# cosmodesi/desilike

Measured on AMD Instinct MI355X. Metric: log-likelihood evals/sec (full-shape P_ell, 3x40 bins), higher is better.
Workload: dtype f64; 1 GPU; BASELINE configs[1]: ShapeFit+Kaiser P_ell ell=(0,2,4) x 40 k-bins, dense window 120x1200 (n_kin=400/ell), 120x120 precision, 1024 batched param points per GPU per step; batch_per_gpu=1024, n_params=6, parallelism=walkers x1, collective=none, ranks=1

## Files before the change

### desilike_amd/csrc/dl_api.hip

```cpp
#include <hip/hip_runtime.h>
#include <chrono>
#include <thread>

#include <algorithm>
#include <cmath>
#include <cstdio>
#include <cstdlib>
#include <string>
#include <vector>

#include "../../include/desilike_amd.h"
#include "dl_host.hpp"
#include "dl_kernels.h"
#include "dl_ens_fold.h"
#include "dl_prior.h"
#include "dl_sample_solved.h"
#include "dl_sample_solved_data.h"
#include "dl_data_batch.h"
#include "dl_data_batch_marg.h"

static thread_local std::string g_last_error;
void dl_set_last_error(const char* msg) { g_last_error = msg ? msg : ""; }

struct DlWhitenHost {
// ... 132 lines not shown
    if (ctx) ctx->last_error = msg;
    g_last_error = msg;
    return 1;
}

template <typename T>
static int dl_upload(dl_ctx* ctx, T** dst, const std::vector<T>& src) {
    size_t bytes = std::max<size_t>(src.size(), 1) * sizeof(T);
    DL_HIP_CHECK(ctx, hipMalloc((void**)dst, bytes));
    if (!src.empty()) DL_HIP_CHECK(ctx, hipMemcpy(*dst, src.data(), src.size() * sizeof(T), hipMemcpyHostToDevice));
    return 0;
}

static_assert(sizeof(DlObsDev) <= 4096, "DlObsDev travels in the kernarg segment (4 KiB)");

extern "C" {

dl_config* dl_config_new(void) { return new dl_config(); }

int dl_config_set_f64(dl_config* cfg, const char* key, const double* data, int64_t n) {
    if (!cfg || !key || (n > 0 && !data) || n < 0) { g_last_error = "dl_config_set_f64: invalid argument"; return 1; }
    cfg->f64[key] = std::vector<double>(data, data + n);
    return 0;
}

int dl_config_set_i32(dl_config* cfg, const char* key, const int32_t* data, int64_t n) {
    if (!cfg || !key || (n > 0 && !data) || n < 0) { g_last_error = "dl_config_set_i32: invalid argument"; return 1; }
    cfg->i32[key] = std::vector<int32_t>(data, data + n);
    return 0;
}
// ... 270 lines not shown
                for (int k = 0; k < K; ++k) sum += wrow[k] * dvec[k];
                tconst[(size_t)s_ * ctx->N_pad + i] = sum;
            }
        }
        if (dl_upload(ctx, &ctx->tconst_dev, tconst)) { dl_destroy(ctx); return 1; }
        ctx->marg.tconst = ctx->tconst_dev;
    }
    if (dl_upload(ctx, &ctx->arena_dev, arena.data)) { dl_destroy(ctx); return 1; }
    for (auto& gf : gfrag_host) {
        double* dev = nullptr;
        if (dl_upload(ctx, &dev, gf)) { dl_destroy(ctx); return 1; }
        ctx->gfrag_dev.push_back(dev);
    }
    ctx->obs_kernarg.resize(ctx->n_obs);
    for (int i = 0; i < ctx->n_obs; ++i) { ctx->obs[i].rebase(ctx->arena_dev); ctx->obs_kernarg[i] = ctx->obs[i].dev; }
    if (dl_upload(ctx, &ctx->obs_array_dev, ctx->obs_kernarg)) { dl_destroy(ctx); return 1; }
    {
        size_t nbytes = (16384 / 32 + 8 + 64) * sizeof(int32_t);
        if (hipMalloc((void**)&ctx->gemm_counters, nbytes) != hipSuccess || hipMemset(ctx->gemm_counters, 0, nbytes) != hipSuccess) { dl_fail(ctx, "dl_create: counter allocation failed"); dl_destroy(ctx); return 1; }
        ctx->step_ready = ctx->gemm_counters + (16384 / 32 + 8);
    }
    {
        std::vector<double> frag((size_t)ctx->N_pad * ctx->K_pad);
        const int nks = ctx->K_pad / 4;
        for (int nt = 0; nt < ctx->N_pad / 16; ++nt)
            for (int ks = 0; ks < nks; ++ks)
                for (int lane = 0; lane < 64; ++lane)
                    frag[((size_t)nt * nks + ks) * 64 + lane] = wt_white[(size_t)(16 * nt + (lane & 15)) * ctx->K_pad + 4 * ks + (lane >> 4)];
        if (dl_upload(ctx, &ctx->wt_frag_dev, frag)) { dl_destroy(ctx); return 1; }
    }
    if (dl_upload(ctx, &ctx->priors_dev, priors) || dl_upload(ctx, &ctx->wt_white_dev, wt_white) ||
// ... 83 lines not shown
    const size_t R = 1 + ctx->n_var;
    DL_HIP_CHECK(ctx, hipMalloc((void**)&ctx->power_ws, (size_t)need * R * ctx->K_pad * sizeof(double)));
    DL_HIP_CHECK(ctx, hipMalloc((void**)&ctx->delta_ws, std::max<size_t>(2 * (size_t)need * R, (size_t)need * R + 16384 + 2048) * ctx->N_pad * sizeof(double)));
    DL_HIP_CHECK(ctx, hipMalloc((void**)&ctx->flat_ws, (size_t)need * ctx->N_pad * sizeof(double)));
    if (ctx->feat_ok) DL_HIP_CHECK(ctx, hipMalloc((void**)&ctx->feat_ws, (size_t)need * ctx->feat_ld * sizeof(double)));
    DL_HIP_CHECK(ctx, hipMalloc((void**)&ctx->stencil_ws, (size_t)need * ctx->n_params * sizeof(double)));
    DL_HIP_CHECK(ctx, hipMalloc((void**)&ctx->prior_rec_ws, (size_t)need * 2 * sizeof(double)));
    if (ctx->ws_ld > 0) {
        DL_HIP_CHECK(ctx, hipMalloc((void**)&ctx->ws_scratch, (size_t)need * ctx->ws_ld * sizeof(double)));
        DL_HIP_CHECK(ctx, hipMemset(ctx->ws_scratch, 0, (size_t)need * ctx->ws_ld * sizeof(double)));
        for (int i = 0; i < ctx->n_obs; ++i) {
            if (ctx->obs[i].dev.templ != 5) continue;
            ctx->obs_kernarg[i].coef_w = ctx->ws_scratch + ctx->obs[i].ws_col;
            ctx->obs_kernarg[i].n_band = (int32_t)ctx->ws_ld;
        }
        DL_HIP_CHECK(ctx, hipMemcpy(ctx->obs_array_dev, ctx->obs_kernarg.data(), ctx->obs_kernarg.size() * sizeof(DlObsDev), hipMemcpyHostToDevice));
    }
    DL_HIP_CHECK(ctx, hipMemset(ctx->power_ws, 0, (size_t)need * R * ctx->K_pad * sizeof(double)));
    DL_HIP_CHECK(ctx, hipMemset(ctx->delta_ws, 0, std::max<size_t>(2 * (size_t)need * R, (size_t)need * R + 16384 + 2048) * ctx->N_pad * sizeof(double)));
    DL_HIP_CHECK(ctx, hipMemset(ctx->flat_ws, 0, (size_t)need * ctx->N_pad * sizeof(double)));
    if (ctx->feat_ok) DL_HIP_CHECK(ctx, hipMemset(ctx->feat_ws, 0, (size_t)need * ctx->feat_ld * sizeof(double)));
    DL_HIP_CHECK(ctx, hipMemset(ctx->stencil_ws, 0, (size_t)need * ctx->n_params * sizeof(double)));
    DL_HIP_CHECK(ctx, hipMemset(ctx->prior_rec_ws, 0, (size_t)need * 2 * sizeof(double)));
    DL_HIP_CHECK(ctx, hipDeviceSynchronize());
    ctx->cap = need;
    return 0;
}

struct DlDataEval {
    const int32_t* index;
    double* out;
// ... 253 lines not shown
    DL_HIP_CHECK(ctx, hipSetDevice(ctx->device));
    if (dl_order_streams(ctx, stream)) return 1;
    const int64_t per_pass = std::max<int64_t>(1, DL_CHUNK / S);
    if (dl_reserve(ctx, std::min<int64_t>(B, per_pass) * S)) return 1;
    for (int64_t b0 = 0; b0 < B; b0 += per_pass) {
        const int64_t nc = std::min<int64_t>(per_pass, B - b0), nb = nc * S;
        const double* steps = steps_dev + (size_t)b0 * P * 2;
        dl_launch_fisher_stencil(centers_dev + (size_t)b0 * P, steps, P, nc, ctx->stencil_ws, stream);
        const double* th = ctx->stencil_ws;
        int n_slabs = 1, cps = 0;
        int64_t slab_stride = 0;
        const double* bias = nullptr;
        const bool emu_fused_env = !dl_options().no_emu_fused;
        const bool emu_fused = emu_fused_env || ctx->any_stacked;
        if (ctx->feat_ok) {
            if (!emu_fused) dl_launch_fullshape(ctx->obs_kernarg.data(), ctx->n_obs, th, P, nb, ctx->power_ws, ctx->K_pad, nullptr, 0, stream, ctx->feat_ws, ctx->feat_ld, 0);
            for (int i = 0; i < ctx->n_obs; ++i) {
                if (ctx->stk_steps[i]) dl_launch_emulated_stacked(ctx->obs_kernarg[i], th, P, nb, ctx->gfrag_dev[i], ctx->delta_ws, ctx->N_pad, ctx->N_pad, i > 0, ctx->stk_steps[i], stream, nullptr, nullptr, nullptr, 0, dl_stk_basis_ws(ctx, i));
                else if (emu_fused) dl_launch_emulated_feature(ctx->obs_kernarg[i], th, P, nb, ctx->gfrag_dev[i], ctx->delta_ws, ctx->N_pad, ctx->N_pad, i > 0, stream);
                else dl_launch_feature_gemm(ctx->feat_ws, ctx->feat_ld, ctx->obs_kernarg[i].feat_off, ctx->obs_kernarg[i].nb_pad, 1, ctx->gfrag_dev[i], ctx->delta_ws, ctx->N_pad,
                                            ctx->N_pad, nb, i > 0, stream);
            }
            bias = ctx->bias_white_dev;
        } else {
            dl_launch_fullshape(ctx->obs_kernarg.data(), ctx->n_obs, th, P, nb, ctx->power_ws, ctx->K_pad, nullptr, 0, stream, nullptr, 0, 0, ctx->obs_array_dev);
            if (ctx->any_transform) {
                dl_launch_window_gemm(ctx->power_ws, ctx->K_pad, ctx->wt_full_dev, ctx->K_pad, ctx->bias_full_dev, ctx->flat_ws, ctx->N_pad, nb, ctx->N_pad, ctx->N_pad, ctx->K_pad, 1, stream);
                dl_launch_transform(ctx->flat_ws, ctx->N_pad, ctx->flatdata_dev, ctx->transform_dev, n, nb, stream);
                dl_launch_window_gemm(ctx->flat_ws, ctx->N_pad, ctx->wh_dev, ctx->N_pad, ctx->bias_wh_dev, ctx->delta_ws, ctx->N_pad, nb, ctx->N_pad, ctx->N_pad, ctx->N_pad, 1, stream);
            } else {
                n_slabs = dl_gemm_tiled_splits(nb, ctx->N_pad, ctx->K_pad, &cps);
// ... 244 lines not shown
        ctx->grad_cap = 0;
        const int64_t cap = std::max<int64_t>((need + 63) / 64 * 64, 256);
        DL_HIP_CHECK(ctx, hipMalloc((void**)&ctx->eg_u, (size_t)cap * K * sizeof(double)));
        DL_HIP_CHECK(ctx, hipMalloc((void**)&ctx->eg_v, (size_t)cap * K * sizeof(double)));
        DL_HIP_CHECK(ctx, hipMalloc((void**)&ctx->eg_q, (size_t)cap * (1 + ctx->n_var) * DL_N_MONO * sizeof(double)));
        DL_HIP_CHECK(ctx, hipMalloc((void**)&ctx->eg_gb, std::max<size_t>(2 * (size_t)cap, (size_t)cap + 16384 + 2048) * ctx->eg_ngt * sizeof(double)));
        DL_HIP_CHECK(ctx, hipMalloc((void**)&ctx->grad_status, (size_t)cap * sizeof(int32_t)));
        DL_HIP_CHECK(ctx, hipMemset(ctx->eg_v, 0, (size_t)cap * K * sizeof(double)));
        DL_HIP_CHECK(ctx, hipDeviceSynchronize());
        ctx->eg_cap = cap;
    }
    for (int64_t b0 = 0; b0 < B; b0 += per_pass) {
        const int64_t nb = std::min<int64_t>(per_pass, B - b0);
        const double* th = theta_dev + (size_t)b0 * P;
        int32_t* st = status_dev ? status_dev + b0 : ctx->grad_status;
        dl_launch_fullshape(ctx->obs_kernarg.data(), 1, th, P, nb, ctx->power_ws, ctx->K_pad, nullptr, 0, stream, ctx->feat_ws, ctx->feat_ld, 0, nullptr);
        dl_launch_emu_grad_u(ctx->feat_ws, ctx->feat_ld, o.feat_off, o.nb_pad, ctx->gfrag_dev[0], ctx->eg_u, Np, Np, nb, stream);
        dl_launch_emu_grad_adjoint(ctx->feat_ws, ctx->feat_ld, o.feat_off, o.nb_pad, ctx->n_var, ctx->eg_u, Np, Np, ctx->bias_white_dev, ctx->marg, th, P, ctx->priors_dev,
                                   logposterior_dev + b0, st, ctx->eg_v, ctx->eg_q, nb, stream);
        int cps = 0;
        const int n_slabs = dl_gemm_tiled_splits(nb, ctx->eg_ngt, (int)K, &cps);
        const int64_t slab_stride = nb * (int64_t)ctx->eg_ngt;
        dl_launch_window_gemm_tiled(ctx->eg_v, K, ctx->eg_gt, K, ctx->eg_gb, slab_stride, ctx->eg_ngt, nb, ctx->eg_ngt, (int)K, n_slabs, cps, stream, 0);
        dl_launch_emu_grad_backprop(o, th, P, ctx->priors_dev, ctx->eg_gb, ctx->eg_ngt, n_slabs, slab_stride, ctx->eg_q, st, ctx->eg_wt, grad_dev + (size_t)b0 * P, nb, stream);
    }
    DL_HIP_CHECK(ctx, hipGetLastError());
    return 0;
}

int dl_eval_logposterior_grad(dl_ctx* ctx, const double* theta_dev, int64_t B, double* logposterior_dev, double* grad_dev, int32_t* status_dev, void* hip_stream) {
    if (!ctx) { g_last_error = "dl_eval_logposterior_grad: null context"; return 1; }
// ... 52 lines not shown
        dl_launch_fullshape_grad(ctx->obs_kernarg.data(), ctx->n_obs, ctx->obs_array_dev, th, P, nb, ctx->grad_y, Kp, ctx->grad_phys, ctx->priors_dev, st, grad_dev + (size_t)b0 * P, stream);
    }
    DL_HIP_CHECK(ctx, hipGetLastError());
    return 0;
}

int dl_eval_theory(dl_ctx* ctx, const double* theta_dev, int64_t B, int32_t iobs, double* power_dev, double* tables_dev, void* hip_stream) {
    if (!ctx) { g_last_error = "dl_eval_theory: null context"; return 1; }
    if (iobs < 0 || iobs >= ctx->n_obs) return dl_fail(ctx, "dl_eval_theory: observable index out of range");
    if (B < 0 || (B > 0 && (!theta_dev || !power_dev))) return dl_fail(ctx, "dl_eval_theory: invalid argument");
    if (B == 0) return 0;
    hipStream_t stream = (hipStream_t)hip_stream;
    DL_HIP_CHECK(ctx, hipSetDevice(ctx->device));
    const bool ws = ctx->obs_kernarg[iobs].templ == 5;
    if (ws && dl_reserve(ctx, B)) return 1;
    DlObsDev tmp = ctx->obs_kernarg[iobs];
    tmp.col_offset = 0;
    tmp.n_pass = 0;
    tmp.n_var = 0;
    for (int c = 0; c < DL_N_VPARS; ++c) tmp.vp_slot[c] = -1;
    for (int c = 0; c < DL_MAX_EFT; ++c) tmp.marg_ct_slot[c][0] = tmp.marg_ct_slot[c][1] = -1;
    if (dl_order_streams(ctx, stream)) return 1;
    for (int64_t b0 = 0, step = ws ? ctx->cap : B; b0 < B; b0 += step)
        dl_launch_fullshape(&tmp, 1, theta_dev + (size_t)b0 * ctx->n_params, ctx->n_params, std::min(step, B - b0), power_dev + (size_t)b0 * tmp.n_in, tmp.n_in,
                            tables_dev ? tables_dev + (size_t)b0 * 3 * tmp.n_in : nullptr, 3 * (int64_t)tmp.n_in, stream);
    DL_HIP_CHECK(ctx, hipGetLastError());
    return 0;
}

int dl_eval_tns_tables(dl_ctx* ctx, const double* theta_dev, int64_t B, int32_t iobs, double* tables_dev, void* hip_stream) {
    if (!ctx) { g_last_error = "dl_eval_tns_tables: null context"; return 1; }
    if (iobs < 0 || iobs >= ctx->n_obs) return dl_fail(ctx, "dl_eval_tns_tables: observable index out of range");
    if (ctx->obs[iobs].dev.theory != 4) return dl_fail(ctx, "dl_eval_tns_tables: the observable's theory is not the TNS model");
    if (B < 0 || (B > 0 && (!theta_dev || !tables_dev))) return dl_fail(ctx, "dl_eval_tns_tables: invalid argument");
    if (B == 0) return 0;
    hipStream_t stream = (hipStream_t)hip_stream;
    DL_HIP_CHECK(ctx, hipSetDevice(ctx->device));
    if (dl_order_streams(ctx, stream)) return 1;
    if (dl_tns_tables(ctx->obs_kernarg[iobs], theta_dev, ctx->n_params, B, tables_dev, stream)) return dl_fail(ctx, std::string("dl_eval_tns_tables: ") + dl_last_error(nullptr));
    DL_HIP_CHECK(ctx, hipGetLastError());
// ... 264 lines not shown
```

### desilike_amd/csrc/dl_kernels.h

```cpp
#pragma once
#include <hip/hip_runtime.h>
#include <hip/hip_ext.h>
#include <stdint.h>

#include "dl_fullshape.h"
#include "dl_prior.h"

struct DlProfEvents { hipEvent_t start = nullptr, stop = nullptr; };
extern thread_local DlProfEvents dl_prof_events;
#define DL_LAUNCH(kernel, grid, block, shm, stream, ...)                                                                                       \
    do {                                                                                                                                       \
        if (dl_prof_events.start) hipExtLaunchKernelGGL(kernel, grid, block, shm, stream, dl_prof_events.start, dl_prof_events.stop, 0, __VA_ARGS__); \
        else hipLaunchKernelGGL(kernel, grid, block, shm, stream, __VA_ARGS__);                                                                \
    } while (0)

struct DlOptions {
    bool no_merged_theory, no_emu_batch, no_fused_solve, no_gram_plain, no_scaled_row0, ef_no_early_theta, fm_no_lane_solve;
    bool chi2_bfrag;
    bool no_stk_split;
    int stk_overlap;
    bool ens_global, ens_force_comm, ens_no_defer, ens_no_fold, ens_stamps, ens_fold_stamps;
    bool no_emu_fused, no_gram_epilogue, step_kernel, chi2_fused, no_chi2_big;
    bool fs_no_moments;
    bool fs_no_prior;
    bool fs_mu_prio;
    int xcd_local;
    long long chi2_max_rows;
    int cg_mt;
    int host_mode;
};
const DlOptions& dl_options();

#define DL_ST_OK 0
#define DL_ST_OUT_OF_PRIOR 1
#define DL_ST_NONFINITE 2
#define DL_ST_NAN_INPUT 3

bool dl_launch_fullshape(const DlObsDev* obs_host, int n_obs, const double* theta, int n_params, int64_t B, double* power, int64_t ld_power, double* tables,
                         int64_t ld_tables, hipStream_t stream, double* feat = nullptr, int64_t feat_ld = 0, int xcd_block = 0,
                         const DlObsDev* obs_dev = nullptr,
// ... 94 lines not shown
```

### desilike_amd/csrc/dl_kernels.hip

```cpp
#include <hip/hip_runtime.h>

#include <algorithm>
#include <cstdio>
#include <cstdlib>
#include <cstring>
#include <vector>

#include "dl_fullshape.h"
#include "dl_wigglesplit.h"
#include <mutex>
#include "dl_kernels.h"
#include "dl_tns.h"
#include "dl_emu_batch.h"
#include "dl_emu_stacked.h"
#include "dl_emu_stacked_ov.h"
#include "dl_emu_stacked_split.h"
#include "dl_finalize_part.h"
#include "dl_marg_solve.h"
#include "dl_scalar_prefetch.h"
#include "dl_ens_fold.h"
#include "dl_fullshape_grad.h"
#include "dl_fullshape_jac.h"

thread_local DlProfEvents dl_prof_events;

__device__ __forceinline__ void dl_obs_prefetch(const void* p) {
    if (__builtin_amdgcn_readfirstlane(threadIdx.x) >= 64) return;
    dl_scalar_prefetch<0, (offsetof(DlObsDev, ct_in) + 63) / 64 * 64, offsetof(DlObsDev, coef_w) / 64 * 64, (sizeof(DlObsDev) + 63) / 64 * 64>(p);
}

static DlOptions g_options;
static std::once_flag g_options_once;
static void dl_options_read() {
    auto on = [](const char* name) { return std::getenv(name) != nullptr; };
    DlOptions& o = g_options;
    o.no_merged_theory = on("DL_NO_MERGED_THEORY"); o.no_emu_batch = on("DL_NO_EMU_BATCH"); o.no_fused_solve = on("DL_NO_FUSED_SOLVE"); o.no_gram_plain = on("DL_NO_GRAM_PLAIN");
    o.no_scaled_row0 = on("DL_NO_SCALED_ROW0"); o.ef_no_early_theta = on("DL_EF_NO_EARLY_THETA"); o.fm_no_lane_solve = on("DL_FM_NO_LANE_SOLVE");
    o.no_stk_split = on("DL_NO_STK_SPLIT");
    o.stk_overlap = std::getenv("DL_STK_OVERLAP") ? atoi(std::getenv("DL_STK_OVERLAP")) : 0;
    o.ens_global = on("DL_ENS_GLOBAL"); o.ens_force_comm = on("DL_ENS_FORCE_COMM"); o.ens_no_defer = on("DL_ENS_NO_DEFER"); o.ens_no_fold = on("DL_ENS_NO_FOLD");
    o.ens_stamps = on("DL_ENS_STAMPS"); o.ens_fold_stamps = on("DL_ENS_FOLD_STAMPS");
    o.cg_mt = std::getenv("DL_CG_MT") ? atoi(std::getenv("DL_CG_MT")) : 0;
    o.host_mode = std::getenv("DL_HOST_MODE") ? atoi(std::getenv("DL_HOST_MODE")) : -1;
    auto flag = [](const char* name) { const char* v = std::getenv(name); return v != nullptr && atoi(v) != 0; };
    o.no_emu_fused = on("DL_NO_EMU_FUSED"); o.no_gram_epilogue = on("DL_NO_GRAM_EPILOGUE"); o.no_chi2_big = on("DL_NO_CHI2_BIG");
    o.fs_no_moments = flag("DL_FS_NO_MOMENTS"); o.fs_no_prior = flag("DL_FS_NO_PRIOR");
    o.fs_mu_prio = std::getenv("DL_FS_MU_PRIO") ? atoi(std::getenv("DL_FS_MU_PRIO")) != 0 : true;
    o.step_kernel = flag("DL_STEP_KERNEL"); o.chi2_fused = flag("DL_CHI2_FUSED"); o.chi2_bfrag = flag("DL_CHI2_BFRAG");
    o.xcd_local = std::getenv("DL_XCD_LOCAL") ? atoi(std::getenv("DL_XCD_LOCAL")) : 1;
    o.chi2_max_rows = std::getenv("DL_CHI2_GEMM_MAX") ? atoll(std::getenv("DL_CHI2_GEMM_MAX")) : 2048;
}
const DlOptions& dl_options() {
    std::call_once(g_options_once, dl_options_read);
    return g_options;
}
extern "C" void dl_options_refresh(void) { (void)dl_options(); dl_options_read(); }

__device__ __forceinline__ int dl_fs_point_of_wg(int wg, int xblk) { return xblk ? xblk * ((wg & 7) + 8 * ((wg >> 3) / xblk)) + ((wg >> 3) % xblk) : wg; }

#define DL_FS_FLAG_PRIO (1 << 16)
#define DL_FS_STAMP_SLOTS 10
#define DL_HWREG_HW_ID ((31 << 11) | 4)
#define DL_HWREG_XCC_ID ((31 << 11) | 20)
static int dl_fs_launch_flags(int xblk, int stop_after) { return stop_after != 0 ? stop_after : (xblk << 8) | (dl_options().fs_mu_prio ? DL_FS_FLAG_PRIO : 0); }

template <bool FAST, int NL, bool EFT, bool DENSE, bool TH_ROW = false, bool SUB = false, int NT = DL_FS_THREADS, bool MOM = false>
__device__ __forceinline__ void dl_fullshape_body(const DlObsDev& o, const double* __restrict__ theta, int n_params, double* __restrict__ power,
                                                  int64_t ld_power, double* __restrict__ tables, int64_t ld_tables, int stop_after, unsigned long long* __restrict__ stamps,
                                                  const double* th_row = nullptr,
                                                  double* lds_sub = nullptr, int tid_sub = 0, int b_sub = 0,
                                                  const DlPriorRec& rec = DlPriorRec{}) {
    extern __shared__ __attribute__((aligned(16))) double lds_wg[];
    double* lds = SUB ? lds_sub : lds_wg;
    const int flags = (SUB || (stop_after & ~0xff) == 0 || stop_after < 0) ? 0 : stop_after;
    const int xblk = (flags >> 8) & 0xff;
    stop_after = (SUB || flags) ? 0 : stop_after;
    const int b = SUB ? b_sub : dl_fs_point_of_wg(blockIdx.x, xblk);
    const int tid = SUB ? tid_sub : (int)threadIdx.x, nthr = NT;
#define DL_STAMP(slot) if (stamps != nullptr && tid == 0) stamps[(size_t)blockIdx.x * DL_FS_STAMP_SLOTS + (slot)] = __builtin_amdgcn_s_memtime();
#define DL_STAMP_HWID(slot) stamps[(size_t)blockIdx.x * DL_FS_STAMP_SLOTS + (slot)] = ((unsigned long long)__builtin_amdgcn_s_getreg(DL_HWREG_XCC_ID) << 32) | __builtin_amdgcn_s_getreg(DL_HWREG_HW_ID);
    DL_STAMP(0)
    if (stamps != nullptr && tid == 0) { stamps[(size_t)blockIdx.x * DL_FS_STAMP_SLOTS + 6] = __builtin_amdgcn_s_memrealtime(); DL_STAMP_HWID(8) }
    if (FAST && stamps != nullptr && tid == NT - 64) { DL_STAMP_HWID(9) }
    const bool toep = !o.fixed_spline && (FAST || o.toeplitz);
    static_assert(!MOM || (FAST && !EFT && !DENSE), "the moment form belongs to the pair evaluation");
    const DlFsShared s = MOM ? dl_fs_shared_carve_mom(lds, o) : dl_fs_shared_carve(lds, o.n_t, o.n_in, dl_fs_n_dd0(o), toep);
    const bool direct = MOM && dl_fs_mom_direct(o);
    const double* th = TH_ROW ? th_row : theta + (size_t)b * n_params;
    if (stop_after == -1) return;
    const bool rec_on = !TH_ROW && rec.lp != nullptr && blockIdx.y == 0, rec_late = FAST && MOM && !o.fixed_spline;
    if (rec_on && !rec_late && __builtin_amdgcn_readfirstlane(tid >> 6) == NT / 64 - 2) dl_prior_record(rec, th, n_params, tid & 63, b);
    double lk_pref[DL_P3_PREF];
#pragma unroll
    for (int it = 0; it < DL_P3_PREF; ++it) lk_pref[it] = (tid + it * nthr < o.n_kin) ? o.lkin[tid + it * nthr] : 0.;
    if (FAST) {
        constexpr int KT = NT - 64;
        const bool mu_wave = tid >= KT;
        constexpr bool PRIO = !SUB && !EFT && !DENSE && NT == DL_FS_THREADS;
        const bool mu_prio = PRIO && (flags & DL_FS_FLAG_PRIO) && __builtin_amdgcn_readfirstlane(tid) >= KT;
        if (mu_prio) __builtin_amdgcn_s_setprio(2);
        const int m = tid - KT;
        const bool mu_lane = mu_wave && m < o.n_mu, scalar_lane = (tid == nthr - 1);
        DlMuCarry c;
        double dlt_pref[DL_TOEP_PREF];
#pragma unroll
        for (int it = 0; it < DL_TOEP_PREF; ++it) dlt_pref[it] = (!MOM && toep && !mu_wave && tid + it * KT < o.n_t - 1) ? o.dlt[tid + it * KT] : 0.;
        const bool knot_rec = MOM && (o.moment_form & 2);
        double kr[DL_KNOT_PREF][2];
#pragma unroll
        for (int it = 0; it < DL_KNOT_PREF; ++it) {
            const bool live = knot_rec && !mu_wave && tid + it * KT < o.n_t;
            const double2 r = live ? *reinterpret_cast<const double2*>(o.knot_rec + 2 * (size_t)(tid + it * KT)) : make_double2(0., 0.);
            kr[it][0] = r.x; kr[it][1] = r.y;
        }
        if (mu_wave) dl_fs_mu_partA(o, th, mu_lane ? m : 0, c);
        else if (knot_rec) dl_fs_knots_rec(tid, KT, o, th, s, kr);
        else dl_fs_knots<!MOM>(tid, KT, o, th, s, b);
        if (o.fixed_spline && mu_wave) {
            dl_fs_mu_partB(c);
            if (mu_lane) dl_fs_mu_partC(o, s, m, c, false);
            if (scalar_lane) dl_fs_scalars(o, th, s, c, false);
        }
        __syncthreads();
        DL_STAMP(1)
        if (stop_after == 1) return;
        if (toep) {
            if (mu_wave) dl_fs_mu_partB(c);
            else dl_fs_phase2_fir<MOM>(tid, KT, o, s);
            __syncthreads();
// ... 50 lines not shown
    if (FAST && !EFT && !DENSE) dl_fs_phase3_pair<NL, EFT, MOM>(tid, nthr, o, s, lk_pref, direct ? prow : nullptr);
    else dl_fs_phase3<FAST, NL, EFT>(tid, nthr, o, s, trow, lk_pref);
    if (!direct) {
        __syncthreads();
        DL_STAMP(4)
        dl_fs_phase4(tid, nthr, o, s, th, prow, ld_power);
    } else {
        DL_STAMP(4)
    }
    DL_STAMP(5)
    if (stamps != nullptr && tid == 0) stamps[(size_t)blockIdx.x * DL_FS_STAMP_SLOTS + 7] = __builtin_amdgcn_s_memrealtime();
#undef DL_STAMP
#undef DL_STAMP_HWID
}

template <bool FAST, int NL, bool EFT, bool DENSE = false, bool MOM = false>
__global__ __launch_bounds__(DL_FS_THREADS, DENSE ? 5 : 4) void dl_fullshape_kernel(const DlObsDev o, const double* __restrict__ theta, int n_params, double* __restrict__ power,
                                                                     int64_t ld_power, double* __restrict__ tables, int64_t ld_tables, int stop_after, unsigned long long* __restrict__ stamps,
                                                                     const DlPriorRec rec) {
    dl_obs_prefetch((const void*)__builtin_amdgcn_kernarg_segment_ptr());
    dl_fullshape_body<FAST, NL, EFT, DENSE, false, false, DL_FS_THREADS, MOM>(o, theta, n_params, power, ld_power, tables, ld_tables, stop_after, stamps, nullptr, nullptr, 0, 0, rec);
}

static bool dl_fs_use_moments(const DlObsDev* obs_host, int n_obs) {
    if (dl_options().fs_no_moments) return false;
    for (int i = 0; i < n_obs; ++i)
        if (!(obs_host[i].moment_form & 1) || obs_host[i].n_ct > 0 || obs_host[i].n_sn > 0) return false;
    return true;
}
static size_t dl_fs_fast_shared_bytes(const DlObsDev& oh, bool mom) { return (mom ? dl_fs_mom_shared_doubles(oh) : dl_fs_shared_doubles_obs(oh, true)) * sizeof(double); }

template <int NL, bool MOM = false>
__global__ __launch_bounds__(512, 2) void dl_fullshape_wide_kernel(const DlObsDev o, const double* __restrict__ theta, int n_params, double* __restrict__ power,
                                                                 int64_t ld_power, int stop_after, unsigned long long* __restrict__ stamps, const DlPriorRec rec) {
    dl_obs_prefetch((const void*)__builtin_amdgcn_kernarg_segment_ptr());
    dl_fullshape_body<true, NL, false, false, false, false, 512, MOM>(o, theta, n_params, power, ld_power, nullptr, 0, stop_after, stamps, nullptr, nullptr, 0, 0, rec);
}


__device__ __forceinline__ void dl_png_build_moments(int tid, int nthr, const DlObsDev& o, const DlFsShared& s, bool toep) {
    if (toep) {
        dl_fs_phase2_fir(tid, nthr, o, s);
    } else {
        dl_fs_phase2a(tid, nthr, o, s);
        __syncthreads();
        dl_fs_phase2b_dot(tid, nthr, o, s);
        __syncthreads();
        dl_fs_phase2b(tid, nthr, o, s);
        __syncthreads();
        dl_fs_phase2c_dot(tid, nthr, o, s);
        __syncthreads();
// ... 20 lines not shown
    __syncthreads();
    dl_png_knots(tid, nthr, o, th, s, false);
    __syncthreads();
    dl_png_build_moments(tid, nthr, o, s, toep);
    dl_png_keep_spline(tid, nthr, o, s, toep, tabs + 2 * n_t, tabs + 3 * n_t);
    __syncthreads();
    dl_png_eval(tid, nthr, o, tabs, murec, sc, s.out);
    __syncthreads();
    double* prow = power + (size_t)b * (1 + o.n_var) * ld_power + o.col_offset;
    for (int idx = tid; idx < o.n_in; idx += nthr) prow[idx] = s.out[idx];
}

template <bool FAST, int NL, bool EFT, bool DENSE = false, bool MOM = false>
__global__ __launch_bounds__(DL_FS_THREADS, DENSE ? 5 : 4) void dl_fullshape_multi_kernel(const DlObsDev* __restrict__ obs, const double* __restrict__ theta, int n_params,
                                                                           double* __restrict__ power, int64_t ld_power, int stop_after, const DlPriorRec rec) {
    dl_fullshape_body<FAST, NL, EFT, DENSE, false, false, DL_FS_THREADS, MOM>(obs[blockIdx.y], theta, n_params, power, ld_power, nullptr, 0, stop_after, nullptr, nullptr, nullptr, 0, 0, rec);
}

#define DL_ENS_MAXP 32
#define DL_ENS_SLOTS_PER_WG 8
#define DL_EF_STAMP(slot) if (f.stamps != nullptr && publish && threadIdx.x == 0) { __builtin_amdgcn_s_waitcnt(0); f.stamps[(size_t)b * 8 + (slot)] = __builtin_amdgcn_s_memtime(); }
__device__ __forceinline__ void dl_ens_propose(const DlEnsFold& f, int b, bool publish, double* __restrict__ th_out, double* __restrict__ scratch) {
#pragma clang fp contract(off)
    const int lane = threadIdx.x & 63;
    DL_EF_STAMP(1)
    const int half = f.nw / 2, P = f.P;
    const DlPhilox r = dl_philox4x32((uint32_t)f.it_prop, (uint32_t)((unsigned long long)f.it_prop >> 32), (uint32_t)b, DL_ENS_STREAM_MOVE + f.half_prop, f.k0, f.k1);
    const double u = dl_uniform53(r.x[0], r.x[1]);
    const double t = (f.a - 1.) * u + 1.;
    const double zz = (t * t) / f.a;
    const int ic = dl_ens_split_at(f.split_prop, (1 - f.half_prop) * half + (int)(r.x[2] % (uint32_t)half));
// ... 403 lines not shown
            else if (model & 32) launch_bao(dl_bao_kernel<3>);
            else if (model & 16) launch_bao(dl_bao_kernel<2>);
            else launch_bao(dl_bao_kernel<1>);
            continue;
        }
        const DlObsDev& oh = obs_host[i];
        const DlPriorRec rec = i == 0 ? rec_on : DlPriorRec{};
        rec_written = rec_written || (i == 0 && rec_ok);
        const bool generic = tables || !oh.uniform_knots || !(oh.toeplitz || oh.fixed_spline);
        static const int64_t dense_min = getenv("DL_FS_DENSE_MIN") ? atoll(getenv("DL_FS_DENSE_MIN")) : 4096;
        bool nl3 = oh.n_ell <= 3, eft = oh.n_ct > 0 || oh.n_sn > 0;
        static const int wide_env = getenv("DL_FS_WIDE") ? atoi(getenv("DL_FS_WIDE")) : -1;
        const bool wide = !generic && !eft && tables == nullptr && (wide_env == 1 || (wide_env != 0 && B * n_obs <= 256));
        const bool mom = moments && !generic && !eft && (wide || B <= dense_min) && dl_fs_use_moments(&oh, 1);
        size_t shmem = generic ? dl_fs_shared_doubles_obs(oh, false) * sizeof(double) : dl_fs_fast_shared_bytes(oh, mom);
        auto launch = [&](auto kernel) {
            if (shmem > 48 * 1024) (void)hipFuncSetAttribute((const void*)kernel, hipFuncAttributeMaxDynamicSharedMemorySize, (int)shmem);
            const int flags = dl_fs_launch_flags((xcd_block > 0 && B % (8 * xcd_block) == 0) ? xcd_block : 0, stop_after);
            DL_LAUNCH(kernel, dim3((unsigned)B), dim3(DL_FS_THREADS), shmem, stream, obs_host[i], theta, n_params, power, ld_power, tables, ld_tables, flags, stamps, rec);
            if (stamps) {
                (void)hipStreamSynchronize(stream);
                std::vector<unsigned long long> h((size_t)B * DL_FS_STAMP_SLOTS);
                (void)hipMemcpy(h.data(), stamps, h.size() * sizeof(unsigned long long), hipMemcpyDeviceToHost);
                if (FILE* f = fopen(stamp_file, "a")) {
                    for (int64_t w = 0; w < B; ++w) { for (int q = 0; q < DL_FS_STAMP_SLOTS; ++q) fprintf(f, "%llu ", h[(size_t)w * DL_FS_STAMP_SLOTS + q]); fprintf(f, "\n"); }
                    fprintf(f, "#\n");
                    fclose(f);
                }
            }
        };
        if (wide) {
            auto launch_wide = [&](auto kernel) {
                if (shmem > 48 * 1024) (void)hipFuncSetAttribute((const void*)kernel, hipFuncAttributeMaxDynamicSharedMemorySize, (int)shmem);
                const int flags = dl_fs_launch_flags((xcd_block > 0 && B % (8 * xcd_block) == 0) ? xcd_block : 0, stop_after);
                DL_LAUNCH(kernel, dim3((unsigned)B), dim3(512), shmem, stream, obs_host[i], theta, n_params, power, ld_power, flags, stamps, rec);
            };
            if (nl3) { if (mom) launch_wide(dl_fullshape_wide_kernel<3, true>); else launch_wide(dl_fullshape_wide_kernel<3>); }
            else { if (mom) launch_wide(dl_fullshape_wide_kernel<5, true>); else launch_wide(dl_fullshape_wide_kernel<5>); }
            continue;
        }
        if (generic) launch(dl_fullshape_kernel<false, 5, true>);
        else if (nl3 && !eft) { if (B > dense_min) launch(dl_fullshape_kernel<true, 3, false, true>); else if (mom) launch(dl_fullshape_kernel<true, 3, false, false, true>); else launch(dl_fullshape_kernel<true, 3, false>); }
        else if (nl3) launch(dl_fullshape_kernel<true, 3, true>);
        else if (!eft) { if (B > dense_min) launch(dl_fullshape_kernel<true, 5, false, true>); else if (mom) launch(dl_fullshape_kernel<true, 5, false, false, true>); else launch(dl_fullshape_kernel<true, 5, false>); }
        else launch(dl_fullshape_kernel<true, 5, true>);
    }
    return rec_written;
}

typedef double dl_double4 __attribute__((ext_vector_type(4)));
typedef double dl_double2 __attribute__((ext_vector_type(2)));

#define DL_GEMM_WAVES 8

struct DlGemmFrag {
    dl_double2 a[4], b0[4], b1[4];
};

__device__ __forceinline__ void dl_gemm_load(DlGemmFrag& f, const double* ap, const double* b0p, const double* b1p, int kc) {
// ... 1153 lines not shown
```

### desilike_amd/csrc/dl_scalar_prefetch.h

```cpp
#pragma once
#include <hip/hip_runtime.h>

template <int A0, int A1, int B0, int B1>
__device__ __forceinline__ void dl_scalar_prefetch(const void* p) {
    __asm__ volatile(
        "s_mov_b32 s83, %1\n"
        "1: s_load_dwordx16 s[84:99], %0, s83\n\ts_add_u32 s83, s83, 64\n\ts_cmp_lt_u32 s83, %2\n\ts_cbranch_scc1 1b\n"
        "s_mov_b32 s83, %3\n"
        "2: s_load_dwordx16 s[84:99], %0, s83\n\ts_add_u32 s83, s83, 64\n\ts_cmp_lt_u32 s83, %4\n\ts_cbranch_scc1 2b\n"
        "s_waitcnt lgkmcnt(0)"
        : : "s"(p), "n"(A0), "n"(A1), "n"(B0), "n"(B1)
        : "s83", "s84", "s85", "s86", "s87", "s88", "s89", "s90", "s91", "s92", "s93", "s94", "s95", "s96", "s97", "s98", "s99", "scc", "memory");
}

template <int BYTES>
__device__ __forceinline__ void dl_kernarg_prefetch() {
    if (__builtin_amdgcn_readfirstlane(threadIdx.x) >= 64) return;
    constexpr int END = (BYTES + 63) / 64 * 64, MID = END > 64 ? 64 : 0;
    dl_scalar_prefetch<0, 64, MID == 0 ? 0 : 64, MID == 0 ? 64 : END>((const void*)__builtin_amdgcn_kernarg_segment_ptr());
}
```

Before: 45.62 million evals/s.

## Pass full-shape observable descriptor by device pointer and hoist early loads

```diff
diff --git a/desilike_amd/csrc/dl_api.hip b/desilike_amd/csrc/dl_api.hip
--- a/desilike_amd/csrc/dl_api.hip
+++ b/desilike_amd/csrc/dl_api.hip
@@ -170,6 +170,21 @@
 
 static_assert(sizeof(DlObsDev) <= 4096, "DlObsDev travels in the kernarg segment (4 KiB)");
 
+static DlObsDev dl_theory_view(const DlObsDev& d) {
+    DlObsDev v = d;
+    v.col_offset = 0;
+    v.n_pass = 0;
+    v.n_var = 0;
+    for (int c = 0; c < DL_N_VPARS; ++c) v.vp_slot[c] = -1;
+    for (int c = 0; c < DL_MAX_EFT; ++c) v.marg_ct_slot[c][0] = v.marg_ct_slot[c][1] = -1;
+    return v;
+}
+static std::vector<DlObsDev> dl_resident_obs(const dl_ctx* ctx) {
+    std::vector<DlObsDev> r(ctx->obs_kernarg);
+    for (const DlObsDev& d : ctx->obs_kernarg) r.push_back(dl_theory_view(d));
+    return r;
+}
+
 extern "C" {
 
 dl_config* dl_config_new(void) { return new dl_config(); }
@@ -470,7 +485,7 @@
     }
     ctx->obs_kernarg.resize(ctx->n_obs);
     for (int i = 0; i < ctx->n_obs; ++i) { ctx->obs[i].rebase(ctx->arena_dev); ctx->obs_kernarg[i] = ctx->obs[i].dev; }
-    if (dl_upload(ctx, &ctx->obs_array_dev, ctx->obs_kernarg)) { dl_destroy(ctx); return 1; }
+    if (dl_upload(ctx, &ctx->obs_array_dev, dl_resident_obs(ctx))) { dl_destroy(ctx); return 1; }
     {
         size_t nbytes = (16384 / 32 + 8 + 64) * sizeof(int32_t);
         if (hipMalloc((void**)&ctx->gemm_counters, nbytes) != hipSuccess || hipMemset(ctx->gemm_counters, 0, nbytes) != hipSuccess) { dl_fail(ctx, "dl_create: counter allocation failed"); dl_destroy(ctx); return 1; }
@@ -584,7 +599,9 @@
             ctx->obs_kernarg[i].coef_w = ctx->ws_scratch + ctx->obs[i].ws_col;
             ctx->obs_kernarg[i].n_band = (int32_t)ctx->ws_ld;
         }
-        DL_HIP_CHECK(ctx, hipMemcpy(ctx->obs_array_dev, ctx->obs_kernarg.data(), ctx->obs_kernarg.size() * sizeof(DlObsDev), hipMemcpyHostToDevice));
+        const std::vector<DlObsDev> resident = dl_resident_obs(ctx);
+        DL_HIP_CHECK(ctx, hipDeviceSynchronize());
+        DL_HIP_CHECK(ctx, hipMemcpy(ctx->obs_array_dev, resident.data(), resident.size() * sizeof(DlObsDev), hipMemcpyHostToDevice));
     }
     DL_HIP_CHECK(ctx, hipMemset(ctx->power_ws, 0, (size_t)need * R * ctx->K_pad * sizeof(double)));
     DL_HIP_CHECK(ctx, hipMemset(ctx->delta_ws, 0, std::max<size_t>(2 * (size_t)need * R, (size_t)need * R + 16384 + 2048) * ctx->N_pad * sizeof(double)));
@@ -868,7 +885,7 @@
         const bool emu_fused_env = !dl_options().no_emu_fused;
         const bool emu_fused = emu_fused_env || ctx->any_stacked;
         if (ctx->feat_ok) {
-            if (!emu_fused) dl_launch_fullshape(ctx->obs_kernarg.data(), ctx->n_obs, th, P, nb, ctx->power_ws, ctx->K_pad, nullptr, 0, stream, ctx->feat_ws, ctx->feat_ld, 0);
+            if (!emu_fused) dl_launch_fullshape(ctx->obs_kernarg.data(), ctx->n_obs, th, P, nb, ctx->power_ws, ctx->K_pad, nullptr, 0, stream, ctx->feat_ws, ctx->feat_ld, 0, ctx->obs_array_dev);
             for (int i = 0; i < ctx->n_obs; ++i) {
                 if (ctx->stk_steps[i]) dl_launch_emulated_stacked(ctx->obs_kernarg[i], th, P, nb, ctx->gfrag_dev[i], ctx->delta_ws, ctx->N_pad, ctx->N_pad, i > 0, ctx->stk_steps[i], stream, nullptr, nullptr, nullptr, 0, dl_stk_basis_ws(ctx, i));
                 else if (emu_fused) dl_launch_emulated_feature(ctx->obs_kernarg[i], th, P, nb, ctx->gfrag_dev[i], ctx->delta_ws, ctx->N_pad, ctx->N_pad, i > 0, stream);
@@ -1143,7 +1160,7 @@
         const int64_t nb = std::min<int64_t>(per_pass, B - b0);
         const double* th = theta_dev + (size_t)b0 * P;
         int32_t* st = status_dev ? status_dev + b0 : ctx->grad_status;
-        dl_launch_fullshape(ctx->obs_kernarg.data(), 1, th, P, nb, ctx->power_ws, ctx->K_pad, nullptr, 0, stream, ctx->feat_ws, ctx->feat_ld, 0, nullptr);
+        dl_launch_fullshape(ctx->obs_kernarg.data(), 1, th, P, nb, ctx->power_ws, ctx->K_pad, nullptr, 0, stream, ctx->feat_ws, ctx->feat_ld, 0, ctx->obs_array_dev);
         dl_launch_emu_grad_u(ctx->feat_ws, ctx->feat_ld, o.feat_off, o.nb_pad, ctx->gfrag_dev[0], ctx->eg_u, Np, Np, nb, stream);
         dl_launch_emu_grad_adjoint(ctx->feat_ws, ctx->feat_ld, o.feat_off, o.nb_pad, ctx->n_var, ctx->eg_u, Np, Np, ctx->bias_white_dev, ctx->marg, th, P, ctx->priors_dev,
                                    logposterior_dev + b0, st, ctx->eg_v, ctx->eg_q, nb, stream);
@@ -1226,16 +1243,11 @@
     DL_HIP_CHECK(ctx, hipSetDevice(ctx->device));
     const bool ws = ctx->obs_kernarg[iobs].templ == 5;
     if (ws && dl_reserve(ctx, B)) return 1;
-    DlObsDev tmp = ctx->obs_kernarg[iobs];
-    tmp.col_offset = 0;
-    tmp.n_pass = 0;
-    tmp.n_var = 0;
-    for (int c = 0; c < DL_N_VPARS; ++c) tmp.vp_slot[c] = -1;
-    for (int c = 0; c < DL_MAX_EFT; ++c) tmp.marg_ct_slot[c][0] = tmp.marg_ct_slot[c][1] = -1;
+    const DlObsDev tmp = dl_theory_view(ctx->obs_kernarg[iobs]);
     if (dl_order_streams(ctx, stream)) return 1;
     for (int64_t b0 = 0, step = ws ? ctx->cap : B; b0 < B; b0 += step)
         dl_launch_fullshape(&tmp, 1, theta_dev + (size_t)b0 * ctx->n_params, ctx->n_params, std::min(step, B - b0), power_dev + (size_t)b0 * tmp.n_in, tmp.n_in,
-                            tables_dev ? tables_dev + (size_t)b0 * 3 * tmp.n_in : nullptr, 3 * (int64_t)tmp.n_in, stream);
+                            tables_dev ? tables_dev + (size_t)b0 * 3 * tmp.n_in : nullptr, 3 * (int64_t)tmp.n_in, stream, nullptr, 0, 0, ctx->obs_array_dev + ctx->n_obs + iobs);
     DL_HIP_CHECK(ctx, hipGetLastError());
     return 0;
 }
diff --git a/desilike_amd/csrc/dl_kernels.h b/desilike_amd/csrc/dl_kernels.h
--- a/desilike_amd/csrc/dl_kernels.h
+++ b/desilike_amd/csrc/dl_kernels.h
@@ -24,6 +24,7 @@
     bool fs_no_moments;
     bool fs_no_prior;
     bool fs_mu_prio;
+    bool fs_desc_kernarg;
     int xcd_local;
     long long chi2_max_rows;
     int cg_mt;
diff --git a/desilike_amd/csrc/dl_kernels.hip b/desilike_amd/csrc/dl_kernels.hip
--- a/desilike_amd/csrc/dl_kernels.hip
+++ b/desilike_amd/csrc/dl_kernels.hip
@@ -27,6 +27,10 @@
 __device__ __forceinline__ void dl_obs_prefetch(const void* p) {
     if (__builtin_amdgcn_readfirstlane(threadIdx.x) >= 64) return;
     dl_scalar_prefetch<0, (offsetof(DlObsDev, ct_in) + 63) / 64 * 64, offsetof(DlObsDev, coef_w) / 64 * 64, (sizeof(DlObsDev) + 63) / 64 * 64>(p);
+}
+__device__ __forceinline__ int dl_obs_prefetch_resident(unsigned long long p) {
+    if (__builtin_amdgcn_readfirstlane(threadIdx.x) >= 64) return 0;
+    return dl_scalar_prefetch_ro<0, (offsetof(DlObsDev, ct_in) + 63) / 64 * 64, offsetof(DlObsDev, coef_w) / 64 * 64, (sizeof(DlObsDev) + 63) / 64 * 64>(p);
 }
 
 static DlOptions g_options;
@@ -46,6 +50,7 @@
     o.no_emu_fused = on("DL_NO_EMU_FUSED"); o.no_gram_epilogue = on("DL_NO_GRAM_EPILOGUE"); o.no_chi2_big = on("DL_NO_CHI2_BIG");
     o.fs_no_moments = flag("DL_FS_NO_MOMENTS"); o.fs_no_prior = flag("DL_FS_NO_PRIOR");
     o.fs_mu_prio = std::getenv("DL_FS_MU_PRIO") ? atoi(std::getenv("DL_FS_MU_PRIO")) != 0 : true;
+    o.fs_desc_kernarg = flag("DL_FS_DESC_KERNARG");
     o.step_kernel = flag("DL_STEP_KERNEL"); o.chi2_fused = flag("DL_CHI2_FUSED"); o.chi2_bfrag = flag("DL_CHI2_BFRAG");
     o.xcd_local = std::getenv("DL_XCD_LOCAL") ? atoi(std::getenv("DL_XCD_LOCAL")) : 1;
     o.chi2_max_rows = std::getenv("DL_CHI2_GEMM_MAX") ? atoll(std::getenv("DL_CHI2_GEMM_MAX")) : 2048;
@@ -64,12 +69,21 @@
 #define DL_HWREG_XCC_ID ((31 << 11) | 20)
 static int dl_fs_launch_flags(int xblk, int stop_after) { return stop_after != 0 ? stop_after : (xblk << 8) | (dl_options().fs_mu_prio ? DL_FS_FLAG_PRIO : 0); }
 
-template <bool FAST, int NL, bool EFT, bool DENSE, bool TH_ROW = false, bool SUB = false, int NT = DL_FS_THREADS, bool MOM = false>
+#define DL_TH_ROW 32
+struct DlFsEarly {
+    const double* knot_rec = nullptr;
+    const double* lkin = nullptr;
+    int n_t = 0, n_kin = 0;
+    unsigned long long desc = 0;
+};
+template <bool FAST, int NL, bool EFT, bool DENSE, bool TH_ROW = false, bool SUB = false, int NT = DL_FS_THREADS, bool MOM = false, bool ROW = false, bool EARLY = false>
 __device__ __forceinline__ void dl_fullshape_body(const DlObsDev& o, const double* __restrict__ theta, int n_params, double* __restrict__ power,
                                                   int64_t ld_power, double* __restrict__ tables, int64_t ld_tables, int stop_after, unsigned long long* __restrict__ stamps,
                                                   const double* th_row = nullptr,
                                                   double* lds_sub = nullptr, int tid_sub = 0, int b_sub = 0,
-                                                  const DlPriorRec& rec = DlPriorRec{}) {
+                                                  const DlPriorRec& rec = DlPriorRec{},
+                                                  const DlFsEarly& early = DlFsEarly{}) {
+    static_assert(!ROW || (FAST && !DENSE && !TH_ROW && !SUB), "the wave-private theta row belongs to the stand-alone fast kernels");
     extern __shared__ __attribute__((aligned(16))) double lds_wg[];
     double* lds = SUB ? lds_sub : lds_wg;
     const int flags = (SUB || (stop_after & ~0xff) == 0 || stop_after < 0) ? 0 : stop_after;
@@ -79,20 +93,49 @@
     const int tid = SUB ? tid_sub : (int)threadIdx.x, nthr = NT;
 #define DL_STAMP(slot) if (stamps != nullptr && tid == 0) stamps[(size_t)blockIdx.x * DL_FS_STAMP_SLOTS + (slot)] = __builtin_amdgcn_s_memtime();
 #define DL_STAMP_HWID(slot) stamps[(size_t)blockIdx.x * DL_FS_STAMP_SLOTS + (slot)] = ((unsigned long long)__builtin_amdgcn_s_getreg(DL_HWREG_XCC_ID) << 32) | __builtin_amdgcn_s_getreg(DL_HWREG_HW_ID);
-    DL_STAMP(0)
-    if (stamps != nullptr && tid == 0) { stamps[(size_t)blockIdx.x * DL_FS_STAMP_SLOTS + 6] = __builtin_amdgcn_s_memrealtime(); DL_STAMP_HWID(8) }
+    const unsigned long long t_entry = __builtin_amdgcn_s_memtime();
+    constexpr bool e_on = EARLY;
+    double th_v = 0.;
+    if (ROW) { const int p = tid & 63; if (p < DL_TH_ROW && p < n_params) th_v = theta[(size_t)b * n_params + p]; }
+    const bool knot_rec = FAST && MOM && (e_on ? early.knot_rec != nullptr : (o.moment_form & 2) != 0);
+    double kr[DL_KNOT_PREF][2];
+    {
+        const double* krp = e_on ? early.knot_rec : o.knot_rec;
+        const int n_t_e = e_on ? early.n_t : o.n_t;
+#pragma unroll
+        for (int it = 0; it < DL_KNOT_PREF; ++it) {
+            const bool live = knot_rec && tid < NT - 64 && tid + it * (NT - 64) < n_t_e;
+            const double2 r = live ? *reinterpret_cast<const double2*>(krp + 2 * (size_t)(tid + it * (NT - 64))) : make_double2(0., 0.);
+            kr[it][0] = r.x; kr[it][1] = r.y;
+        }
+    }
+    double lk_pref[DL_P3_PREF];
+    {
+        const double* lkp = e_on ? early.lkin : o.lkin;
+        const int n_kin_e = e_on ? early.n_kin : o.n_kin;
+#pragma unroll
+        for (int it = 0; it < DL_P3_PREF; ++it) lk_pref[it] = (tid + it * nthr < n_kin_e) ? lkp[tid + it * nthr] : 0.;
+    }
+    const int pf_zero = EARLY ? dl_obs_prefetch_resident(early.desc) : 0;
+    if (stamps != nullptr && tid == 0) { stamps[(size_t)blockIdx.x * DL_FS_STAMP_SLOTS + 0] = t_entry; stamps[(size_t)blockIdx.x * DL_FS_STAMP_SLOTS + 6] = __builtin_amdgcn_s_memrealtime(); DL_STAMP_HWID(8) }
     if (FAST && stamps != nullptr && tid == NT - 64) { DL_STAMP_HWID(9) }
     const bool toep = !o.fixed_spline && (FAST || o.toeplitz);
     static_assert(!MOM || (FAST && !EFT && !DENSE), "the moment form belongs to the pair evaluation");
     const DlFsShared s = MOM ? dl_fs_shared_carve_mom(lds, o) : dl_fs_shared_carve(lds, o.n_t, o.n_in, dl_fs_n_dd0(o), toep);
     const bool direct = MOM && dl_fs_mom_direct(o);
-    const double* th = TH_ROW ? th_row : theta + (size_t)b * n_params;
+    const double* th = TH_ROW ? th_row : theta + (size_t)b * n_params + (ROW ? 0 : pf_zero);
+    if (ROW) {
+        __shared__ double dl_th_rows[(NT / 64) * DL_TH_ROW];
+        double* row = dl_th_rows + __builtin_amdgcn_readfirstlane(tid >> 6) * DL_TH_ROW + pf_zero;
+        if ((tid & 63) < DL_TH_ROW) row[tid & 63] = th_v;
+        __builtin_amdgcn_fence(__ATOMIC_RELEASE, "wavefront");
+        __builtin_amdgcn_wave_barrier();
+        __builtin_amdgcn_fence(__ATOMIC_ACQUIRE, "wavefront");
+        if (n_params <= DL_TH_ROW) th = row;
+    }
     if (stop_after == -1) return;
     const bool rec_on = !TH_ROW && rec.lp != nullptr && blockIdx.y == 0, rec_late = FAST && MOM && !o.fixed_spline;
     if (rec_on && !rec_late && __builtin_amdgcn_readfirstlane(tid >> 6) == NT / 64 - 2) dl_prior_record(rec, th, n_params, tid & 63, b);
-    double lk_pref[DL_P3_PREF];
-#pragma unroll
-    for (int it = 0; it < DL_P3_PREF; ++it) lk_pref[it] = (tid + it * nthr < o.n_kin) ? o.lkin[tid + it * nthr] : 0.;
     if (FAST) {
         constexpr int KT = NT - 64;
         const bool mu_wave = tid >= KT;
@@ -105,14 +148,6 @@
         double dlt_pref[DL_TOEP_PREF];
 #pragma unroll
         for (int it = 0; it < DL_TOEP_PREF; ++it) dlt_pref[it] = (!MOM && toep && !mu_wave && tid + it * KT < o.n_t - 1) ? o.dlt[tid + it * KT] : 0.;
-        const bool knot_rec = MOM && (o.moment_form & 2);
-        double kr[DL_KNOT_PREF][2];
-#pragma unroll
-        for (int it = 0; it < DL_KNOT_PREF; ++it) {
-            const bool live = knot_rec && !mu_wave && tid + it * KT < o.n_t;
-            const double2 r = live ? *reinterpret_cast<const double2*>(o.knot_rec + 2 * (size_t)(tid + it * KT)) : make_double2(0., 0.);
-            kr[it][0] = r.x; kr[it][1] = r.y;
-        }
         if (mu_wave) dl_fs_mu_partA(o, th, mu_lane ? m : 0, c);
         else if (knot_rec) dl_fs_knots_rec(tid, KT, o, th, s, kr);
         else dl_fs_knots<!MOM>(tid, KT, o, th, s, b);
@@ -193,12 +228,28 @@
 #undef DL_STAMP_HWID
 }
 
+#define DL_FS_PTR_ARGS const DlObsDev* __restrict__ obs, const double* __restrict__ theta, const double* __restrict__ knot_rec, const double* __restrict__ lkin,                   \
+                       unsigned long long obs_addr, int n_params, int stop_after, int sizes, double* __restrict__ power, double* __restrict__ rec_lp,                          \
+                       int32_t* __restrict__ rec_flag, const double* __restrict__ rec_priors, int64_t ld_power
+__device__ __forceinline__ DlFsEarly dl_fs_early(unsigned long long obs_addr, const double* knot_rec, const double* lkin, int sizes) {
+    DlFsEarly e;
+    e.knot_rec = knot_rec; e.lkin = lkin; e.n_t = sizes & 0xffff; e.n_kin = (sizes >> 16) & 0xffff; e.desc = obs_addr;
+    return e;
+}
+__device__ __forceinline__ DlPriorRec dl_fs_rec(const double* priors, double* lp, int32_t* flag) { DlPriorRec r; r.priors = priors; r.lp = lp; r.flag = flag; return r; }
+
 template <bool FAST, int NL, bool EFT, bool DENSE = false, bool MOM = false>
-__global__ __launch_bounds__(DL_FS_THREADS, DENSE ? 5 : 4) void dl_fullshape_kernel(const DlObsDev o, const double* __restrict__ theta, int n_params, double* __restrict__ power,
-                                                                     int64_t ld_power, double* __restrict__ tables, int64_t ld_tables, int stop_after, unsigned long long* __restrict__ stamps,
-                                                                     const DlPriorRec rec) {
+__global__ __launch_bounds__(DL_FS_THREADS, DENSE ? 5 : 4) void dl_fullshape_kernel(DL_FS_PTR_ARGS, double* __restrict__ tables, int64_t ld_tables, unsigned long long* __restrict__ stamps) {
+    dl_fullshape_body<FAST, NL, EFT, DENSE, false, false, DL_FS_THREADS, MOM, FAST && !DENSE, true>(*obs, theta, n_params, power, ld_power, tables, ld_tables, stop_after, stamps, nullptr, nullptr, 0, 0,
+                                                                                             dl_fs_rec(rec_priors, rec_lp, rec_flag), dl_fs_early(obs_addr, knot_rec, lkin, sizes));
+}
+
+template <int NL>
+__global__ __launch_bounds__(DL_FS_THREADS, 4) void dl_fullshape_byval_kernel(const DlObsDev o, const double* __restrict__ theta, int n_params, double* __restrict__ power,
+                                                                             int64_t ld_power, double* __restrict__ tables, int64_t ld_tables, int stop_after, unsigned long long* __restrict__ stamps,
+                                                                             const DlPriorRec rec) {
     dl_obs_prefetch((const void*)__builtin_amdgcn_kernarg_segment_ptr());
-    dl_fullshape_body<FAST, NL, EFT, DENSE, false, false, DL_FS_THREADS, MOM>(o, theta, n_params, power, ld_power, tables, ld_tables, stop_after, stamps, nullptr, nullptr, 0, 0, rec);
+    dl_fullshape_body<true, NL, false, false, false, false, DL_FS_THREADS, true>(o, theta, n_params, power, ld_power, tables, ld_tables, stop_after, stamps, nullptr, nullptr, 0, 0, rec);
 }
 
 static bool dl_fs_use_moments(const DlObsDev* obs_host, int n_obs) {
@@ -210,10 +261,9 @@
 static size_t dl_fs_fast_shared_bytes(const DlObsDev& oh, bool mom) { return (mom ? dl_fs_mom_shared_doubles(oh) : dl_fs_shared_doubles_obs(oh, true)) * sizeof(double); }
 
 template <int NL, bool MOM = false>
-__global__ __launch_bounds__(512, 2) void dl_fullshape_wide_kernel(const DlObsDev o, const double* __restrict__ theta, int n_params, double* __restrict__ power,
-                                                                 int64_t ld_power, int stop_after, unsigned long long* __restrict__ stamps, const DlPriorRec rec) {
-    dl_obs_prefetch((const void*)__builtin_amdgcn_kernarg_segment_ptr());
-    dl_fullshape_body<true, NL, false, false, false, false, 512, MOM>(o, theta, n_params, power, ld_power, nullptr, 0, stop_after, stamps, nullptr, nullptr, 0, 0, rec);
+__global__ __launch_bounds__(512, 2) void dl_fullshape_wide_kernel(DL_FS_PTR_ARGS, unsigned long long* __restrict__ stamps) {
+    dl_fullshape_body<true, NL, false, false, false, false, 512, MOM, true, true>(*obs, theta, n_params, power, ld_power, nullptr, 0, stop_after, stamps, nullptr, nullptr, 0, 0,
+                                                                           dl_fs_rec(rec_priors, rec_lp, rec_flag), dl_fs_early(obs_addr, knot_rec, lkin, sizes));
 }
 
 
@@ -264,7 +314,7 @@
 template <bool FAST, int NL, bool EFT, bool DENSE = false, bool MOM = false>
 __global__ __launch_bounds__(DL_FS_THREADS, DENSE ? 5 : 4) void dl_fullshape_multi_kernel(const DlObsDev* __restrict__ obs, const double* __restrict__ theta, int n_params,
                                                                            double* __restrict__ power, int64_t ld_power, int stop_after, const DlPriorRec rec) {
-    dl_fullshape_body<FAST, NL, EFT, DENSE, false, false, DL_FS_THREADS, MOM>(obs[blockIdx.y], theta, n_params, power, ld_power, nullptr, 0, stop_after, nullptr, nullptr, nullptr, 0, 0, rec);
+    dl_fullshape_body<FAST, NL, EFT, DENSE, false, false, DL_FS_THREADS, MOM, FAST && !DENSE>(obs[blockIdx.y], theta, n_params, power, ld_power, nullptr, 0, stop_after, nullptr, nullptr, nullptr, 0, 0, rec);
 }
 
 #define DL_ENS_MAXP 32
@@ -698,35 +748,50 @@
         const bool wide = !generic && !eft && tables == nullptr && (wide_env == 1 || (wide_env != 0 && B * n_obs <= 256));
         const bool mom = moments && !generic && !eft && (wide || B <= dense_min) && dl_fs_use_moments(&oh, 1);
         size_t shmem = generic ? dl_fs_shared_doubles_obs(oh, false) * sizeof(double) : dl_fs_fast_shared_bytes(oh, mom);
+        if (obs_dev == nullptr || oh.n_t > 0xffff || oh.n_kin > 0xffff) {
+            dl_set_last_error("dl_launch_fullshape: the full-shape theory kernels read the observable's description from the context's device array (none was passed)");
+            fprintf(stderr, "desilike_amd: dl_launch_fullshape without a device description: launch skipped\n");
+            continue;
+        }
+        const int flags = dl_fs_launch_flags((xcd_block > 0 && B % (8 * xcd_block) == 0) ? xcd_block : 0, stop_after);
+        const int sizes = oh.n_t | (oh.n_kin << 16);
+        const double* knot_rec_e = (mom && (oh.moment_form & 2)) ? oh.knot_rec : nullptr;
+        auto dump_stamps = [&]() {
+            if (!stamps) return;
+            (void)hipStreamSynchronize(stream);
+            std::vector<unsigned long long> h((size_t)B * DL_FS_STAMP_SLOTS);
+            (void)hipMemcpy(h.data(), stamps, h.size() * sizeof(unsigned long long), hipMemcpyDeviceToHost);
+            if (FILE* f = fopen(stamp_file, "a")) {
+                for (int64_t w = 0; w < B; ++w) { for (int q = 0; q < DL_FS_STAMP_SLOTS; ++q) fprintf(f, "%llu ", h[(size_t)w * DL_FS_STAMP_SLOTS + q]); fprintf(f, "\n"); }
+                fprintf(f, "#\n");
+                fclose(f);
+            }
+        };
         auto launch = [&](auto kernel) {
             if (shmem > 48 * 1024) (void)hipFuncSetAttribute((const void*)kernel, hipFuncAttributeMaxDynamicSharedMemorySize, (int)shmem);
-            const int flags = dl_fs_launch_flags((xcd_block > 0 && B % (8 * xcd_block) == 0) ? xcd_block : 0, stop_after);
+            DL_LAUNCH(kernel, dim3((unsigned)B), dim3(DL_FS_THREADS), shmem, stream, obs_dev + i, theta, knot_rec_e, oh.lkin, (unsigned long long)(uintptr_t)(obs_dev + i), n_params, flags, sizes, power, rec.lp, rec.flag, rec.priors, ld_power,
+                      tables, ld_tables, stamps);
+            dump_stamps();
+        };
+        auto launch_byval = [&](auto kernel) {
+            if (shmem > 48 * 1024) (void)hipFuncSetAttribute((const void*)kernel, hipFuncAttributeMaxDynamicSharedMemorySize, (int)shmem);
             DL_LAUNCH(kernel, dim3((unsigned)B), dim3(DL_FS_THREADS), shmem, stream, obs_host[i], theta, n_params, power, ld_power, tables, ld_tables, flags, stamps, rec);
-            if (stamps) {
-                (void)hipStreamSynchronize(stream);
-                std::vector<unsigned long long> h((size_t)B * DL_FS_STAMP_SLOTS);
-                (void)hipMemcpy(h.data(), stamps, h.size() * sizeof(unsigned long long), hipMemcpyDeviceToHost);
-                if (FILE* f = fopen(stamp_file, "a")) {
-                    for (int64_t w = 0; w < B; ++w) { for (int q = 0; q < DL_FS_STAMP_SLOTS; ++q) fprintf(f, "%llu ", h[(size_t)w * DL_FS_STAMP_SLOTS + q]); fprintf(f, "\n"); }
-                    fprintf(f, "#\n");
-                    fclose(f);
-                }
-            }
+            dump_stamps();
         };
+        const bool byval = dl_options().fs_desc_kernarg;
         if (wide) {
             auto launch_wide = [&](auto kernel) {
                 if (shmem > 48 * 1024) (void)hipFuncSetAttribute((const void*)kernel, hipFuncAttributeMaxDynamicSharedMemorySize, (int)shmem);
-                const int flags = dl_fs_launch_flags((xcd_block > 0 && B % (8 * xcd_block) == 0) ? xcd_block : 0, stop_after);
-                DL_LAUNCH(kernel, dim3((unsigned)B), dim3(512), shmem, stream, obs_host[i], theta, n_params, power, ld_power, flags, stamps, rec);
+                DL_LAUNCH(kernel, dim3((unsigned)B), dim3(512), shmem, stream, obs_dev + i, theta, knot_rec_e, oh.lkin, (unsigned long long)(uintptr_t)(obs_dev + i), n_params, flags, sizes, power, rec.lp, rec.flag, rec.priors, ld_power, stamps);
             };
             if (nl3) { if (mom) launch_wide(dl_fullshape_wide_kernel<3, true>); else launch_wide(dl_fullshape_wide_kernel<3>); }
             else { if (mom) launch_wide(dl_fullshape_wide_kernel<5, true>); else launch_wide(dl_fullshape_wide_kernel<5>); }
             continue;
         }
         if (generic) launch(dl_fullshape_kernel<false, 5, true>);
-        else if (nl3 && !eft) { if (B > dense_min) launch(dl_fullshape_kernel<true, 3, false, true>); else if (mom) launch(dl_fullshape_kernel<true, 3, false, false, true>); else launch(dl_fullshape_kernel<true, 3, false>); }
+        else if (nl3 && !eft) { if (B > dense_min) launch(dl_fullshape_kernel<true, 3, false, true>); else if (mom && byval) launch_byval(dl_fullshape_byval_kernel<3>); else if (mom) launch(dl_fullshape_kernel<true, 3, false, false, true>); else launch(dl_fullshape_kernel<true, 3, false>); }
         else if (nl3) launch(dl_fullshape_kernel<true, 3, true>);
-        else if (!eft) { if (B > dense_min) launch(dl_fullshape_kernel<true, 5, false, true>); else if (mom) launch(dl_fullshape_kernel<true, 5, false, false, true>); else launch(dl_fullshape_kernel<true, 5, false>); }
+        else if (!eft) { if (B > dense_min) launch(dl_fullshape_kernel<true, 5, false, true>); else if (mom && byval) launch_byval(dl_fullshape_byval_kernel<5>); else if (mom) launch(dl_fullshape_kernel<true, 5, false, false, true>); else launch(dl_fullshape_kernel<true, 5, false>); }
         else launch(dl_fullshape_kernel<true, 5, true>);
     }
     return rec_written;
diff --git a/desilike_amd/csrc/dl_scalar_prefetch.h b/desilike_amd/csrc/dl_scalar_prefetch.h
--- a/desilike_amd/csrc/dl_scalar_prefetch.h
+++ b/desilike_amd/csrc/dl_scalar_prefetch.h
@@ -12,6 +12,20 @@
         : : "s"(p), "n"(A0), "n"(A1), "n"(B0), "n"(B1)
         : "s83", "s84", "s85", "s86", "s87", "s88", "s89", "s90", "s91", "s92", "s93", "s94", "s95", "s96", "s97", "s98", "s99", "scc", "memory");
 }
+template <int A0, int A1, int B0, int B1>
+__device__ __forceinline__ int dl_scalar_prefetch_ro(unsigned long long addr) {
+    int zero;
+    __asm__(
+        "s_mov_b32 s83, %2\n"
+        "1: s_load_dwordx16 s[84:99], %1, s83\n\ts_add_u32 s83, s83, 64\n\ts_cmp_lt_u32 s83, %3\n\ts_cbranch_scc1 1b\n"
+        "s_mov_b32 s83, %4\n"
+        "2: s_load_dwordx16 s[84:99], %1, s83\n\ts_add_u32 s83, s83, 64\n\ts_cmp_lt_u32 s83, %5\n\ts_cbranch_scc1 2b\n"
+        "s_waitcnt lgkmcnt(0)\n"
+        "s_mov_b32 %0, 0"
+        : "=s"(zero) : "s"(addr), "n"(A0), "n"(A1), "n"(B0), "n"(B1)
+        : "s83", "s84", "s85", "s86", "s87", "s88", "s89", "s90", "s91", "s92", "s93", "s94", "s95", "s96", "s97", "s98", "s99", "scc");
+    return zero;
+}
 
 template <int BYTES>
 __device__ __forceinline__ void dl_kernarg_prefetch() {
```

Result: no change. 45.98 million evals/s (median of 6 runs) (+0.8%).
